# chao-ji/ldm_tf2

Hardware: AMD Instinct MI355X
Metric: images/sec (256x256, 200 DDIM steps, CFG=5) (higher is better)
Workload: dtype bf16

## Files before the change

ldm_tf2_amd/csrc/gemm.hip:

```cpp
#include "gemm_kernel.h"
#include "gemm3_kernel.h"
#include "gemm_tiles.h"

using namespace ldm_gemm_detail;

namespace {

__global__ __launch_bounds__(256) void splitk_epilogue_kernel(GemmArgs p) {
  const int nout = p.act == LDM_ACT_GEGLU ? p.N / 2 : p.N;
  const int64_t total = (int64_t)p.M * nout;
  for (int64_t idx = (int64_t)blockIdx.x * 256 + threadIdx.x; idx < total;
       idx += (int64_t)gridDim.x * 256) {
    const int m = (int)(idx / nout), c = (int)(idx - (int64_t)m * nout);
    if (p.act == LDM_ACT_GEGLU) {
      const int nv = (c >> 5) * 64 + (c & 31), ng = nv + 32;
      float a = 0.f, g = 0.f;
      for (int s = 0; s < p.split_k; ++s) {
        const float* ws = p.ws + ((int64_t)s * p.M + m) * p.N;
        a += ws[nv]; g += ws[ng];
      }
      epi_store(p, 0, m, c, epi_pre(p, m, nv, a) * gelu_erf_f(epi_pre(p, m, ng, g)));
    } else {
      float a = 0.f;
      for (int s = 0; s < p.split_k; ++s) a += p.ws[((int64_t)s * p.M + m) * p.N + c];
// ... 147 lines not shown
                        (p->split_k <= 0 && (!p->workspace || (size_t)split * p->M * p->N * 4 > p->workspace_bytes))))
        continue;
      const int kps = cdiv(ktiles, split);
      const double rounds = (double)(int64_t)((tiles * split + 256.0 * t.resident - 1) / (256.0 * t.resident));
      double us = rounds * (kps + t.overhead_steps) * t.step_us * f32x;
      if (!no_t2pref && t.prefer_over &&
          (double)m_tiles(p, kTiles[t.prefer_over].bm) * cdiv(p->N, kTiles[t.prefer_over].bn) * p->batch < 256.0)
        us *= kCoResidentPreference;
      if (split > 1) us += 3.0 + (double)p->M * p->N * 4.0 * (split + 1) / 3.0e6;
      if (us < best) { best = us; best_cfg = c; best_split = split; }
    }
  }
  if (p->split_k > 0 && p->batch == 1) best_split = p->split_k;
  const int twin = kTiles[best_cfg].halo_twin;
  if (tile_given) best_cfg = p->tile;
  else if (twin && halo_ring_ok(p) && p->N % kTiles[twin].bn == 0 && !p->out2 && !p->ln_out && !p->a2 &&
           ktiles / best_split >= kHaloTwinMinKtiles)
    best_cfg = twin;
  return {best_cfg, best_split, 0};
}

Plan final_plan(const ldm_gemm_params* p) {
  const int esize = elem_size(p);
  auto [cfg, split, kps] = choose(p, esize);
  if (p->ln_out) { cfg = kLnTile; split = 1; }
  if (p->ln_cs && !has(cfg, tPers)) {
    const bool wide_ok = p->act != LDM_ACT_GEGLU && p->N % kTiles[kLnFoldWideTile].bn == 0;
    cfg = wide_ok && (p->N % kTiles[kLnFoldTile].bn != 0 || p->tile == kLnFoldWideTile) ? kLnFoldWideTile : kLnFoldTile;
    split = 1;
  }
  if (p->out2 || has(cfg, tPers)) split = 1;
  const int ktiles = cdiv(p->K, 128 / esize);
  kps = cdiv(ktiles, split < 1 ? 1 : split);
  if (has(cfg, tHalo)) kps = cdiv(kps, 9) * 9;
  return {cfg, cdiv(ktiles, kps), kps};
}

int64_t a_extent(const ldm_gemm_params* p, int cols) {
  return (p->conv ? ((int64_t)p->B * p->H * p->W - 1) * p->lda + p->Cin : ((int64_t)p->M - 1) * p->lda + cols) * elem_size(p);
}
int64_t w_extent(const ldm_gemm_params* p) { return (int64_t)p->N * p->K * elem_size(p); }

template <typename Args>
Args common_args(const ldm_gemm_params* p) {
  Args a;
  memset(&a, 0, sizeof(a));
  a.a = (const char*)p->a; a.w = (const char*)p->w; a.bias = p->bias; a.addend = p->addend;
  a.residual = (const char*)p->residual; a.out = (char*)p->out;
  a.lda = p->lda; a.ldr = p->ldr; a.add_ld = p->add_ld; a.M = p->M; a.N = p->N; a.K = p->K;
  a.a_bytes = (uint32_t)a_extent(p, p->K - (p->a2 ? p->Cin2 : 0)); a.w_bytes = (uint32_t)w_extent(p);
  a.add_rows = p->add_rows > 0 ? p->add_rows : 1;
  a.conv = p->conv; a.H = p->H; a.W = p->W; a.Cin = p->Cin; a.OH = p->OH; a.OW = p->OW;
  a.stride = p->stride; a.upsample = p->upsample; a.pad = p->no_lead_pad ? 0 : 1; a.act = p->act;
  return a;
}

GemmArgs build_args(const ldm_gemm_params* p, Plan pl) {
  const int esize = elem_size(p), bke = 128 / esize;
  GemmArgs a = common_args<GemmArgs>(p);
  a.ws = (float*)p->workspace; a.ldc_m = p->ldc_m; a.ldc_n = p->ldc_n; a.batch = p->batch;
  a.stride_a = p->stride_a; a.stride_w = p->stride_w; a.stride_c = p->stride_c; a.stride_r = p->stride_r;
  a.out_dtype = p->out_dtype; a.alpha = p->alpha;
  a.ln_out = (char*)p->ln_out; a.ln_gamma = p->ln_gamma; a.ln_beta = p->ln_beta; a.ld_ln = p->ld_ln; a.ln_eps = p->ln_eps;
  a.out2 = (char*)p->out2; a.ld2 = p->ld2; a.stride2 = p->stride2; a.n_split = p->n_split; a.rows2 = p->rows2;
  a.ktiles = a.kt9 = cdiv(p->K, bke);
  if (p->a2) {
    a.a2 = (const char*)p->a2; a.lda2 = p->lda2; a.kt9 = (p->K - p->Cin2) / bke;
    a.a2_bytes = (uint32_t)((((int64_t)p->M - 1) * p->lda2 + p->Cin2) * esize);
  }
  a.vec_epilogue = vec_epilogue_ok(p);
  a.split_k = pl.split; a.ktiles_per_split = pl.kps;
  a.tiles_m = m_tiles(p, kTiles[pl.cfg].bm); a.tiles_n = cdiv(p->N, kTiles[pl.cfg].bn);
#ifdef LDM_TOOLS_BUILD
  { static const bool adj = getenv("LDM_UP2_PHASE_ADJACENT") != nullptr; a.phase_adjacent = adj; }
#endif
  return a;
}

int launch_reduce(const ldm_gemm_params* p, const GemmArgs& a, hipStream_t s) {
  const int nout = p->act == LDM_ACT_GEGLU ? p->N / 2 : p->N;
  const bool vec = a.vec_epilogue && ((uintptr_t)p->workspace % 16) == 0 && p->N % 4 == 0;
  int64_t total = vec ? (int64_t)p->M * (nout / 8) : (int64_t)p->M * nout;
  int blocks = (int)((total + 255) / 256);
  if (blocks > 4096) blocks = 4096;
  if (vec) hipLaunchKernelGGL(splitk_epilogue_vec_kernel, dim3(blocks), dim3(256), 0, s, a);
  else hipLaunchKernelGGL(splitk_epilogue_kernel, dim3(blocks), dim3(256), 0, s, a);
  return ldm_launch_status("ldm_gemm(splitk epilogue)");
}

int check_shape(const ldm_gemm_params* p) {
  LDM_CHECK_ARG(p && p->a && p->w && p->out, "ldm_gemm: null pointer");
  LDM_CHECK_ARG(p->dtype == LDM_F32 || p->dtype == LDM_BF16, "ldm_gemm: bad dtype %d", p->dtype);
  LDM_CHECK_ARG(p->out_dtype == LDM_F32 || p->out_dtype == LDM_BF16, "ldm_gemm: bad out_dtype");
  LDM_CHECK_ARG(p->M > 0 && p->N > 0 && p->K > 0 && p->batch > 0, "ldm_gemm: bad M/N/K/batch");
  const int esize = elem_size(p);
  const int epc = 16 / esize, bke = 8 * epc;
  LDM_CHECK_ARG(p->K % bke == 0, "ldm_gemm: K=%d must be a multiple of the K-tile (%d elements)", p->K, bke);
  LDM_CHECK_ARG(((uintptr_t)p->a % 16) == 0 && ((uintptr_t)p->w % 16) == 0,
                "ldm_gemm: a/w must be 16-byte aligned");
  LDM_CHECK_ARG(p->lda % epc == 0 && p->stride_a % epc == 0 && p->stride_w % epc == 0,
                "ldm_gemm: lda/stride_a/stride_w must be multiples of %d elements", epc);
  if (p->conv) {
    LDM_CHECK_ARG(p->Cin > 0 && p->Cin % bke == 0, "ldm_gemm(conv): Cin=%d must be a multiple of %d",
                  p->Cin, bke);
    if (p->upsample == 2) {
      LDM_CHECK_ARG(p->K == 4 * p->Cin, "ldm_gemm(conv): the phase form (upsample = 2) needs K == 4*Cin (K=%d Cin=%d)", p->K, p->Cin);
// ... 228 lines not shown
```

ldm_tf2_amd/csrc/gemm3_kernel.h:

```cpp
#pragma once
#include "gemm_kernel.h"

namespace ldm_gemm_detail {

struct Gemm3Args {
  const char* a;
  const char* w;
  const float* bias;
  const float* addend;
  const char* residual;
  char* out;
  int64_t lda, ldr, ldc, add_ld;
  uint32_t a_bytes, w_bytes;
  int M, N, K;
  int add_rows;
  int conv, H, W, Cin, OH, OW, stride, upsample, pad;
  int act;
  int ktiles;
  int panels;
  int ntiles;
  int nsplit;
  int tiles_per_wg;
  char* out_t;
  int64_t ld_t, stride_t;
  int rows_t;
  int n_split;
  int ntiles1;
  const float* ln_cs;
  float ln_eps;
#ifdef LDM_TOOLS_BUILD
  int dbg;
#endif
};

#ifdef LDM_TOOLS_BUILD
#define LDM_G3_DBG(p) ((p).dbg)
#else
#define LDM_G3_DBG(p) 0
#endif

constexpr int kEpiBias = 1, kEpiAdd = 2, kEpiRes = 4, kEpiTrans = 32, kEpiLn = 64, kEpiSplit = 128;
constexpr int epi_code(bool bias, bool add, bool res, int act) { return (bias ? 1 : 0) | (add ? 2 : 0) | (res ? 4 : 0) | (act << 3); }

#if defined(__HIP_DEVICE_COMPILE__)
template <int TN, int MODE, int EPI, bool TR>
__device__ __forceinline__ void gemm3_body(const Gemm3Args& p, char* smem, const int panel, const int nt_begin, const int ntl) {
  constexpr int BM = 256, BN = 32 * TN, WM = 4, WN = 2, NW = 8;
  constexpr int WTM = 64, WTN = 16 * TN, TM = 4;
  constexpr int NIB = BN / 8;
  constexpr int LA = BM / (8 * NW), LB = (NIB + NW - 1) / NW, LBF = NIB / NW;
  constexpr int NL = LA + LB;
  constexpr int ES = 2;
  constexpr int STAGE = (BM + BN) * 128;
  constexpr int NSTAGE = 3;
  constexpr int LNX = (EPI & 64) ? NW * 64 * 8 : 0;
  static_assert(NSTAGE * STAGE + LNX <= 160 * 1024, "LDS");
  typedef __attribute__((address_space(3))) void* lds_ptr;

  const int tid = threadIdx.x;
  const int lane = tid & 63;
  const int wave = __builtin_amdgcn_readfirstlane(tid >> 6);
  const int wm = wave / WN, wn = wave % WN;
  const int m0 = panel * BM;
  const int nk = p.ktiles;
  const int S = ntl * nk;

  const __amdgpu_buffer_rsrc_t rsA =
      __builtin_amdgcn_make_buffer_rsrc(const_cast<char*>(p.a), 0, p.a_bytes, 0x00020000);
  const __amdgpu_buffer_rsrc_t rsW =
      __builtin_amdgcn_make_buffer_rsrc(const_cast<char*>(p.w), 0, p.w_bytes, 0x00020000);

  int a_base[LA], a_mask[LA], a_aux[LA];
#pragma unroll
  for (int i = 0; i < LA; ++i) {
    const int row = (i * NW + wave) * 8 + (lane >> 3);
    const int ck = (lane & 7) ^ ((row >> 1) & 7);
    const int m = m0 + row;
    a_base[i] = MODE == 0 ? (int)kOOB : 0; a_mask[i] = 0; a_aux[i] = 0;
    if (m < p.M) {
      if constexpr (MODE != 0) {
        const int ohw = p.OH * p.OW;
        const int b = m / ohw, rem = m - b * ohw;
        const int oy = rem / p.OW, ox = rem - oy * p.OW;
        const int iy0 = oy * p.stride - p.pad, ix0 = ox * p.stride - p.pad;
// ... 134 lines not shown
                                                                __builtin_bit_cast(bf16x8, fb[kg][j]), acc[i][j], 0, 0, 0);
          else
            acc[i][j] = __builtin_amdgcn_mfma_f32_16x16x32_bf16(__builtin_bit_cast(bf16x8, fb[kg][j]),
                                                                __builtin_bit_cast(bf16x8, fa[kg][i]), acc[i][j], 0, 0, 0);
        }
    __builtin_amdgcn_s_setprio(0);
  };

  [[maybe_unused]] float ln_s = 0.f, ln_q = 0.f;
  [[maybe_unused]] auto ln_accum = [&](const char* cS) {
    if constexpr ((EPI & kEpiLn) != 0) {
      typedef __bf16 bf2 __attribute__((ext_vector_type(2)));
      const int row = wm * WTM + lane;
      const char* base = cS + row * 128;
      const int rot = row >> 1;
      const bf2 one = __builtin_bit_cast(bf2, 0x3f803f80u);
#pragma unroll
      for (int j = 0; j < 8; j += 2) {
        const u32x4 c0 = *(const u32x4*)(base + (((j + rot) & 7) << 4));
        const u32x4 c1 = *(const u32x4*)(base + (((j + 1 + rot) & 7) << 4));
#pragma unroll
        for (int e = 0; e < 4; ++e) {
          const uint32_t w0 = c0[e], w1 = c1[e];
          const bf2 a0 = __builtin_bit_cast(bf2, w0), a1 = __builtin_bit_cast(bf2, w1);
          ln_s = __builtin_amdgcn_fdot2_f32_bf16(a0, one, ln_s, false);
          ln_q = __builtin_amdgcn_fdot2_f32_bf16(a0, a0, ln_q, false);
          ln_s = __builtin_amdgcn_fdot2_f32_bf16(a1, one, ln_s, false);
          ln_q = __builtin_amdgcn_fdot2_f32_bf16(a1, a1, ln_q, false);
        }
      }
    }
  };

  [[maybe_unused]] auto ln_publish = [&]() {
    if constexpr ((EPI & kEpiLn) != 0) {
      ldm_f32x2 v = {ln_s, ln_q};
      *(ldm_f32x2*)(smem + NSTAGE * STAGE + (wave * 64 + lane) * 8) = v;
      asm volatile("s_waitcnt lgkmcnt(0)" ::: "memory");
    }
  };
  [[maybe_unused]] auto ln_combine = [&]() {
    if constexpr ((EPI & kEpiLn) != 0) {
      const ldm_f32x2 o = *(const ldm_f32x2*)(smem + NSTAGE * STAGE + ((wave ^ 1) * 64 + lane) * 8);
      ln_s += o[0]; ln_q += o[1];
    }
  };

  constexpr bool HB = (EPI & kEpiBias) != 0, HA = (EPI & kEpiAdd) != 0, HR = (EPI & kEpiRes) != 0;
  constexpr int ACT = (EPI >> 3) & 3;
  constexpr bool LN = (EPI & kEpiLn) != 0;
  static_assert(!LN || (MODE == 0 && HB), "LayerNorm fold: plain rows, with the folded bias");
  constexpr bool GEGLU = ACT == LDM_ACT_GEGLU;
  static_assert(!GEGLU || TN == 4, "GEGLU: the wave tile must be one 64-row block of the interleaved weights");
  auto epilogue = [&](int tl) {
    if (LDM_G3_DBG(p) & 2) return;
    const int n_w = (nt_begin + tl) * BN + wn * WTN;
    const int g = lh;
    [[maybe_unused]] float ln_mu = 0.f, ln_r = 0.f;
    if constexpr (LN) {
      const float ik = 1.0f / (float)p.K;
      ln_mu = ln_s * ik;
      const float ex2 = ln_q * ik;
      ln_r = rsqrtf(fmaxf(__builtin_fmaf(-ln_mu, ln_mu, ex2), 0.f) + p.ln_eps);
    }
    if constexpr (TR) {
      const int n_t = SPLIT ? n_w - p.n_split : n_w;
      const int col2 = lane >> 2, pc = lane & 3;
      const int src = (16 * ((pc >> 1) | ((pc & 1) << 1)) + col2) * 4;
#pragma unroll
      for (int ip = 0; ip < TM; ip += 2) {
        const int mrow = m0 + wm * WTM + 16 * ip + 8 * pc;
        const bool valid = mrow < p.M && !(LDM_G3_DBG(p) & 1);
        const int mc = valid ? mrow : 0;
        const int smp = mc / p.rows_t, tok = mc - smp * p.rows_t;
        bf16_t* obase = (bf16_t*)p.out_t + (int64_t)smp * p.stride_t + tok;
        [[maybe_unused]] float rmu[2][4], rrs[2][4];
        if constexpr (LN) {
#pragma unroll
          for (int h = 0; h < 2; ++h)
#pragma unroll
            for (int r = 0; r < 4; ++r) {
              rmu[h][r] = __shfl(ln_mu, 16 * (ip + h) + 4 * g + r, 64);
              rrs[h][r] = __shfl(ln_r, 16 * (ip + h) + 4 * g + r, 64);
            }
        }
#pragma unroll
        for (int j = 0; j < TN; ++j) {
          if constexpr (LN) {
            const float cs = p.ln_cs[n_w + 16 * j + lr], bb = p.bias[n_w + 16 * j + lr];
#pragma unroll
            for (int h = 0; h < 2; ++h)
#pragma unroll
              for (int r = 0; r < 4; ++r)
                acc[ip + h][j][r] = __builtin_fmaf(rrs[h][r], acc[ip + h][j][r], __builtin_fmaf(-rrs[h][r] * rmu[h][r], cs, bb));
          }
          const uint32_t x0 = pack_bf2(acc[ip][j][0], acc[ip][j][1]), x1 = pack_bf2(acc[ip][j][2], acc[ip][j][3]);
          const uint32_t y0 = pack_bf2(acc[ip + 1][j][0], acc[ip + 1][j][1]), y1 = pack_bf2(acc[ip + 1][j][2], acc[ip + 1][j][3]);
          const auto s0 = __builtin_amdgcn_permlane16_swap(x0, y0, false, false);
          const auto s1 = __builtin_amdgcn_permlane16_swap(x1, y1, false, false);
          u32x4 o;
          o[0] = (uint32_t)__builtin_amdgcn_ds_bpermute(src, (int)s0[0]);
          o[1] = (uint32_t)__builtin_amdgcn_ds_bpermute(src, (int)s1[0]);
          o[2] = (uint32_t)__builtin_amdgcn_ds_bpermute(src, (int)s0[1]);
          o[3] = (uint32_t)__builtin_amdgcn_ds_bpermute(src, (int)s1[1]);
          if (valid) *(u32x4*)(obase + (int64_t)(n_t + 16 * j + col2) * p.ld_t) = o;
        }
      }
      return;
    }
    f32x4 bv[TN];
    if constexpr (HB) {
#pragma unroll
      for (int j = 0; j < TN; ++j) bv[j] = *(const f32x4*)(p.bias + n_w + 16 * j + 4 * g);
    }
    [[maybe_unused]] f32x4 csv[TN];
    if constexpr (LN) {
#pragma unroll
      for (int j = 0; j < TN; ++j) csv[j] = *(const f32x4*)(p.ln_cs + n_w + 16 * j + 4 * g);
    }
    constexpr int NOB = GEGLU ? TN / 2 : TN;
    const int n_o = GEGLU ? (n_w >> 1) : n_w;
    [[maybe_unused]] u32x2 rva[TM][NOB];
    if constexpr (HR) {
#pragma unroll
      for (int i = 0; i < TM; ++i) {
        const int m = m0 + wm * WTM + 16 * i + lr;
        const bf16_t* rr = (const bf16_t*)p.residual + (int64_t)(m < p.M ? m : p.M - 1) * p.ldr + n_o + 4 * g;
#pragma unroll
        for (int j = 0; j < NOB; ++j) rva[i][j] = *(const u32x2*)(rr + 16 * j);
      }
    }
#pragma unroll
    for (int i = 0; i < TM; ++i) {
      const int m = m0 + wm * WTM + 16 * i + lr;
      const bool valid = m < p.M;
      const int mc = valid ? m : p.M - 1;
      f32x4 av[TN];
      if constexpr (HA) {
        const float* ad = p.addend + (int64_t)(mc / p.add_rows) * p.add_ld + n_w + 4 * g;
#pragma unroll
        for (int j = 0; j < TN; ++j) av[j] = *(const f32x4*)(ad + 16 * j);
      }
      u32x2 rv[NOB];
      if constexpr (HR) {
#pragma unroll
        for (int j = 0; j < NOB; ++j) rv[j] = rva[i][j];
      }
      [[maybe_unused]] float mu_i = 0.f, rs_i = 0.f;
      [[maybe_unused]] float nm_i = 0.f;
      if constexpr (LN) {
        mu_i = __shfl(ln_mu, 16 * i + lr, 64);
        rs_i = __shfl(ln_r, 16 * i + lr, 64);
        nm_i = -rs_i * mu_i;
      }
      auto block = [&](int j, float (&v)[4]) {
#pragma unroll
        for (int r = 0; r < 4; ++r) v[r] = acc[i][j][r];
        if constexpr (LN) {
#pragma unroll
          for (int r = 0; r < 4; ++r) v[r] = __builtin_fmaf(rs_i, v[r], __builtin_fmaf(nm_i, csv[j][r], bv[j][r]));
        } else if constexpr (HB) {
#pragma unroll
          for (int r = 0; r < 4; ++r) v[r] += bv[j][r];
        }
        if constexpr (HA) {
#pragma unroll
          for (int r = 0; r < 4; ++r) v[r] += av[j][r];
        }
      };
      auto finish = [&](int jo, float (&v)[4], uint32_t (&pk)[2]) {
        if constexpr (HR) {
          v[0] += __uint_as_float(rv[jo][0] << 16); v[1] += __uint_as_float(rv[jo][0] & 0xffff0000u);
          v[2] += __uint_as_float(rv[jo][1] << 16); v[3] += __uint_as_float(rv[jo][1] & 0xffff0000u);
        }
        pk[0] = pack_bf2(v[0], v[1]);
        pk[1] = pack_bf2(v[2], v[3]);
      };
      uint32_t pk[NOB][2];
      if constexpr (GEGLU) {
#pragma unroll
        for (int j = 0; j < 2; ++j) {
          float v[4], gt[4];
          block(j, v);
// ... 6 lines not shown
#pragma unroll
        for (int j = 0; j < TN; ++j) {
          float v[4];
          block(j, v);
          if constexpr (ACT == LDM_ACT_GELU) {
#pragma unroll
            for (int r = 0; r < 4; ++r) v[r] = gelu_erf_f(v[r]);
          } else if constexpr (ACT == LDM_ACT_SILU) {
#pragma unroll
            for (int r = 0; r < 4; ++r) v[r] = silu_f(v[r]);
          }
          finish(j, v, pk[j]);
        }
      }
      const int row2 = lane >> 2, pc = lane & 3;
      const int src = (16 * ((pc >> 1) | ((pc & 1) << 1)) + row2) * 4;
      const int m2 = m0 + wm * WTM + 16 * i + row2;
      const bool valid2 = m2 < p.M && !(LDM_G3_DBG(p) & 1);
      bf16_t* orow2 = (bf16_t*)p.out + (int64_t)(valid2 ? m2 : 0) * p.ldc + n_o;
#pragma unroll
      for (int j = 0; j + 1 < NOB; j += 2) {
        const auto s0 = __builtin_amdgcn_permlane16_swap(pk[j][0], pk[j + 1][0], false, false);
        const auto s1 = __builtin_amdgcn_permlane16_swap(pk[j][1], pk[j + 1][1], false, false);
        u32x4 o;
        o[0] = (uint32_t)__builtin_amdgcn_ds_bpermute(src, (int)s0[0]);
        o[1] = (uint32_t)__builtin_amdgcn_ds_bpermute(src, (int)s1[0]);
        o[2] = (uint32_t)__builtin_amdgcn_ds_bpermute(src, (int)s0[1]);
        o[3] = (uint32_t)__builtin_amdgcn_ds_bpermute(src, (int)s1[1]);
        if (valid2) *(u32x4*)(orow2 + 16 * j + 8 * pc) = o;
      }
      if constexpr (NOB & 1) {
        const int src1 = (16 * pc + row2) * 4;
        u32x2 o;
        o[0] = (uint32_t)__builtin_amdgcn_ds_bpermute(src1, (int)pk[NOB - 1][0]);
        o[1] = (uint32_t)__builtin_amdgcn_ds_bpermute(src1, (int)pk[NOB - 1][1]);
        if (valid2) *(u32x2*)(orow2 + 16 * (NOB - 1) + 4 * pc) = o;
      }
    }
  };

  int is_tl = 0, is_kt = 0;
  auto issue_next = [&](int stage) {
    if (!(LDM_G3_DBG(p) & 8)) issue_tile(is_tl, is_kt, stage);
    if (++is_kt == nk) { is_kt = 0; ++is_tl; }
  };
  issue_next(0);
  if (S > 1) issue_next(1);
  int st = 0, ck = 0, ctl = 0;
  const bool late = wave >= NW / 2;
  auto wait_step = [&](int s) {
    if (s + 1 < S && (LDM_G3_DBG(p) & 16)) {
      if (b_last) asm volatile("s_waitcnt vmcnt(%0)" ::"n"(LB) : "memory");
      else asm volatile("s_waitcnt vmcnt(%0)" ::"n"(LB - 1) : "memory");
    } else if (s + 1 < S) {
      if (b_last) asm volatile("s_waitcnt vmcnt(%0)" ::"n"(NL) : "memory");
      else asm volatile("s_waitcnt vmcnt(%0)" ::"n"(NL - 1) : "memory");
    } else {
      asm volatile("s_waitcnt vmcnt(0)" ::: "memory");
    }
  };
  if (!late) {
    for (int s = 0; s < S; ++s) {
      wait_step(s);
      __builtin_amdgcn_s_barrier();
      if constexpr (LN) { if (s == nk) ln_combine(); }
      if (ck == 0 && s > 0) { epilogue(ctl - 1); zero_acc(); }
      int sn = st + 2; sn = sn >= NSTAGE ? sn - NSTAGE : sn;
      if (s + 2 < S) issue_next(sn);
      read_frags(smem + st * STAGE);
      if constexpr (LN) {
        if (ctl == 0) {
          if ((ck & 1) == wn) ln_accum(smem + st * STAGE);
          if (ck == nk - 1) ln_publish();
        }
      }
      multiply(0);
      st = st + 1 == NSTAGE ? 0 : st + 1;
      if (++ck == nk) { ck = 0; ++ctl; }
    }
  } else {
    for (int s = 0; s < S; ++s) {
      wait_step(s);
      __builtin_amdgcn_s_barrier();
      if (s > 0) multiply(1);
      if constexpr (LN) { if (s == nk) ln_combine(); }
      if (ck == 0 && s > 0) { epilogue(ctl - 1); zero_acc(); }
      int sn = st + 2; sn = sn >= NSTAGE ? sn - NSTAGE : sn;
      if (s + 2 < S) issue_next(sn);
      read_frags(smem + st * STAGE);
      if constexpr (LN) {
        if (ctl == 0) {
          if ((ck & 1) == wn) ln_accum(smem + st * STAGE);
          if (ck == nk - 1) ln_publish();
        }
      }
      st = st + 1 == NSTAGE ? 0 : st + 1;
      if (++ck == nk) { ck = 0; ++ctl; }
      asm volatile("s_waitcnt lgkmcnt(0)" ::: "memory");
      __builtin_amdgcn_sched_barrier(0);
    }
    multiply(1);
  }
  if constexpr (LN) {
    if (ntl == 1) {
      __builtin_amdgcn_s_barrier();
      ln_combine();
    }
  }
  epilogue(ntl - 1);
}
#endif

template <int TN, int MODE, int EPI>
__global__ __launch_bounds__(512) void gemm3_kernel(Gemm3Args p) {
#if defined(__HIP_DEVICE_COMPILE__)
  constexpr int BM = 256, BN = 32 * TN;
  constexpr int LNX = (EPI & 64) ? 8 * 64 * 8 : 0;
  __shared__ __attribute__((aligned(16))) char smem[3 * (BM + BN) * 128 + LNX];
  int bid = blockIdx.x;
  {
    const int nwg = gridDim.x;
    const int q = nwg >> 3, r = nwg & 7, x = bid & 7;
    bid = (x < r ? x * (q + 1) : r * (q + 1) + (x - r) * q) + (bid >> 3);
  }
  const int panel = bid / p.nsplit, sp = bid - panel * p.nsplit;
  if constexpr ((EPI & kEpiSplit) != 0) {
    const int nt_begin = sp * p.tiles_per_wg;
    const int nt_end = min(p.ntiles, nt_begin + p.tiles_per_wg);
    const int a_end = min(nt_end, p.ntiles1);
    if (nt_begin < a_end) gemm3_body<TN, MODE, EPI, false>(p, smem, panel, nt_begin, a_end - nt_begin);
    const int b_begin = max(nt_begin, p.ntiles1);
    if (b_begin < nt_end) {
      if (nt_begin < a_end) __syncthreads();
      gemm3_body<TN, MODE, EPI, true>(p, smem, panel, b_begin, nt_end - b_begin);
    }
  } else {
    const int nt_begin = sp * p.tiles_per_wg;
    const int ntl = min(p.ntiles, nt_begin + p.tiles_per_wg) - nt_begin;
    if (ntl > 0)
      gemm3_body<TN, MODE, EPI, (EPI & kEpiTrans) != 0>(p, smem, panel, nt_begin, ntl);
  }
#endif
}

template <int MODE>
bool launch_gemm3(int tn, int epi, const Gemm3Args& a, dim3 grid, hipStream_t s);
bool launch_gemm3_ln(int tn, int epi, const Gemm3Args& a, dim3 grid, hipStream_t s);

}
```

ldm_tf2_amd/csrc/gemm_kernel.h:

```cpp
#pragma once
#include "common.h"
#include <stdlib.h>

namespace ldm_gemm_detail {


struct GemmArgs {
  const char* a;
  const char* w;
  const float* bias;
  const float* addend;
  const char* residual;
  char* out;
  float* ws;
  int64_t lda, ldr, ldc_m, ldc_n;
  int64_t stride_a, stride_w, stride_c, stride_r;
  int64_t add_ld;
  uint32_t a_bytes, w_bytes;
  int M, N, K, batch;
  int add_rows;
  int conv, H, W, Cin, OH, OW, stride, upsample, pad;
  int act, out_dtype;
  int split_k, ktiles_per_split, ktiles;
  int tiles_m, tiles_n;
  int vec_epilogue;
  float alpha;
  char* ln_out;
  const float* ln_gamma;
  const float* ln_beta;
  int64_t ld_ln;
  float ln_eps;
  char* out2;
  int64_t ld2, stride2;
  int n_split, rows2;
  const char* a2;
  int64_t lda2;
  uint32_t a2_bytes;
  int kt9;
  int phase_adjacent;
};

constexpr uint32_t kOOB = 0x80000000u;

__device__ __forceinline__ void mma32(f32x16& acc, const u32x4& a, const u32x4& b, bf16_t) {
  acc = __builtin_amdgcn_mfma_f32_32x32x16_bf16(__builtin_bit_cast(bf16x8, a),
                                                __builtin_bit_cast(bf16x8, b), acc, 0, 0, 0);
}
__device__ __forceinline__ void mma32(f32x16& acc, const u32x4& a, const u32x4& b, float) {
#pragma unroll
  for (int j = 0; j < 4; ++j)
    acc = __builtin_amdgcn_mfma_f32_32x32x2f32(__uint_as_float(a[j]), __uint_as_float(b[j]), acc,
                                               0, 0, 0);
}

__device__ __forceinline__ uint32_t pick6(int j, uint32_t a0, uint32_t a1, uint32_t a2, uint32_t a3, uint32_t a4, uint32_t a5) {
  uint32_t v = a0;
  v = j == 1 ? a1 : v;
  v = j == 2 ? a2 : v;
  v = j == 3 ? a3 : v;
  v = j == 4 ? a4 : v;
  v = j == 5 ? a5 : v;
  return v;
}

__device__ __forceinline__ float epi_pre(const GemmArgs& p, int m, int n, float acc) {
  float v = acc * p.alpha;
  if (p.bias) v += p.bias[n];
  if (p.addend) v += p.addend[(int64_t)(m / p.add_rows) * p.add_ld + n];
  return v;
}

__device__ __forceinline__ void epi_store(const GemmArgs& p, int bz, int m, int ncol, float v) {
  const int64_t off = (int64_t)bz * p.stride_c + (int64_t)m * p.ldc_m + (int64_t)ncol * p.ldc_n;
  if (p.out_dtype == LDM_BF16) {
    if (p.residual)
      v += bf2f(((const bf16_t*)p.residual)[(int64_t)bz * p.stride_r + (int64_t)m * p.ldr + ncol]);
    ((bf16_t*)p.out)[off] = f2bf(v);
  } else {
    if (p.residual)
      v += ((const float*)p.residual)[(int64_t)bz * p.stride_r + (int64_t)m * p.ldr + ncol];
    ((float*)p.out)[off] = v;
  }
}

__device__ __forceinline__ float apply_act(int act, float v) {
  if (act == LDM_ACT_GELU) return gelu_erf_f(v);
  if (act == LDM_ACT_SILU) return silu_f(v);
  return v;
}

template <typename T, int BM, int BN, int WM, int WN, int MODE, int MF = 0, int ST = 0, int NS = 0>
__global__ __launch_bounds__(WM* WN * 64) void gemm_kernel(GemmArgs p) {
#if defined(__HIP_DEVICE_COMPILE__)
// ... 441 lines not shown
#pragma unroll
          for (int e = 0; e < 4; ++e)
            v[e] = apply_act(p.act, epi_pre(p, min(m + e, p.M - 1), n, acc[i][j][r4 * 4 + e]));
          const int64_t off = (int64_t)(m / p.rows2) * p.stride2 + (int64_t)(n - p.n_split) * p.ld2 + (m % p.rows2);
          if (p.out_dtype == LDM_BF16) {
            u32x2 pk; pk[0] = pack_bf2(v[0], v[1]); pk[1] = pack_bf2(v[2], v[3]);
            *(u32x2*)((bf16_t*)p.out2 + off) = pk;
          } else {
            f32x4 pk = {v[0], v[1], v[2], v[3]};
            *(f32x4*)((float*)p.out2 + off) = pk;
          }
        }
      }
    return;
  }
  if (p.split_k > 1) {
    float* ws = p.ws + (int64_t)split * p.M * p.N;
#pragma unroll
    for (int i = 0; i < TM; ++i)
#pragma unroll
      for (int j = 0; j < TN; ++j) {
        const int n = nb + j * MB;
        if (n >= p.N) continue;
#pragma unroll
        for (int r = 0; r < NR; ++r) {
          const int m = mb + i * MB + rowoff(r);
          if (m < Mrows) ws[(int64_t)orow(m) * p.N + n] = acc[i][j][r];
        }
      }
    return;
  }

  if (p.vec_epilogue) {
    float* sC = (float*)smem;
    const bool geglu = p.act == LDM_ACT_GEGLU;
    constexpr int PCOLS = BN / 8;
    const int pcols = geglu ? PCOLS / 2 : PCOLS;
    const int npieces = EROWS * pcols;
    const int nout = geglu ? p.N / 2 : (p.out2 ? p.n_split : p.N);
#pragma unroll
   for (int ep = 0; ep < ESPLIT; ++ep) {
    if (ep > 0) __syncthreads();
    if ((wm * WTM) / EROWS == ep) {
#pragma unroll
      for (int i = 0; i < TM; ++i)
#pragma unroll
        for (int j = 0; j < TN; ++j)
#pragma unroll
          for (int r = 0; r < NR; ++r) {
            const int row = wm * WTM - ep * EROWS + i * MB + rowoff(r) + 4 * lh;
            sC[row * BN + wn * WTN + j * MB + lr] = acc[i][j][r] * p.alpha;
          }
    }
    __syncthreads();
    for (int c = tid; c < npieces; c += NT) {
      const int row = c / pcols, pc = c - row * pcols;
      int m = m0 + ep * EROWS + row;
      int ncol, lcol;
      if (geglu) {
        const int oc = pc * 8;
        lcol = (oc >> 5) * 64 + (oc & 31);
        ncol = (n0 >> 1) + oc;
      } else {
        lcol = pc * 8;
        ncol = n0 + lcol;
      }
      if (m >= Mrows || ncol >= nout) continue;
      m = orow(m);
      float v[8];
      {
        const f32x4 x0 = *(const f32x4*)(sC + row * BN + lcol);
        const f32x4 x1 = *(const f32x4*)(sC + row * BN + lcol + 4);
#pragma unroll
        for (int e = 0; e < 4; ++e) { v[e] = x0[e]; v[4 + e] = x1[e]; }
      }
      const int nlog = geglu ? n0 + lcol : ncol;
      if (p.bias) {
        const f32x4 b0 = *(const f32x4*)(p.bias + nlog), b1 = *(const f32x4*)(p.bias + nlog + 4);
#pragma unroll
        for (int e = 0; e < 4; ++e) { v[e] += b0[e]; v[4 + e] += b1[e]; }
      }
      if (p.addend) {
        const float* ad = p.addend + (int64_t)(m / p.add_rows) * p.add_ld + nlog;
        const f32x4 a0 = *(const f32x4*)ad, a1 = *(const f32x4*)(ad + 4);
#pragma unroll
        for (int e = 0; e < 4; ++e) { v[e] += a0[e]; v[4 + e] += a1[e]; }
      }
      if (geglu) {
        float g[8];
        const f32x4 x0 = *(const f32x4*)(sC + row * BN + lcol + 32);
        const f32x4 x1 = *(const f32x4*)(sC + row * BN + lcol + 36);
#pragma unroll
        for (int e = 0; e < 4; ++e) { g[e] = x0[e]; g[4 + e] = x1[e]; }
        if (p.bias) {
          const f32x4 b0 = *(const f32x4*)(p.bias + nlog + 32), b1 = *(const f32x4*)(p.bias + nlog + 36);
#pragma unroll
          for (int e = 0; e < 4; ++e) { g[e] += b0[e]; g[4 + e] += b1[e]; }
        }
#pragma unroll
        for (int e = 0; e < 8; ++e) v[e] *= gelu_erf_f(g[e]);
      } else if (p.act != LDM_ACT_NONE) {
#pragma unroll
        for (int e = 0; e < 8; ++e) v[e] = apply_act(p.act, v[e]);
      }
      const int64_t ooff = (int64_t)bz * p.stride_c + (int64_t)m * p.ldc_m + ncol;
      const int64_t roff = (int64_t)bz * p.stride_r + (int64_t)m * p.ldr + ncol;
      if (p.out_dtype == LDM_BF16) {
        if (p.residual) {
          float rr[8];
          chunk_to_f32(*(const u32x4*)((const bf16_t*)p.residual + roff), rr, bf16_t());
#pragma unroll
          for (int e = 0; e < 8; ++e) v[e] += rr[e];
        }
        *(u32x4*)((bf16_t*)p.out + ooff) = f32_to_chunk(v, bf16_t());
      } else {
        if (p.residual) {
          const f32x4 r0 = *(const f32x4*)((const float*)p.residual + roff);
          const f32x4 r1 = *(const f32x4*)((const float*)p.residual + roff + 4);
#pragma unroll
          for (int e = 0; e < 4; ++e) { v[e] += r0[e]; v[4 + e] += r1[e]; }
        }
        f32x4 o0 = {v[0], v[1], v[2], v[3]}, o1 = {v[4], v[5], v[6], v[7]};
        *(f32x4*)((float*)p.out + ooff) = o0;
        *(f32x4*)((float*)p.out + ooff + 4) = o1;
      }
      if (p.ln_out) {
        if (p.out_dtype == LDM_BF16) {
#pragma unroll
          for (int e = 0; e < 8; ++e) v[e] = bf2f(f2bf(v[e]));
        }
        f32x4 o0 = {v[0], v[1], v[2], v[3]}, o1 = {v[4], v[5], v[6], v[7]};
        *(f32x4*)(sC + row * BN + lcol) = o0;
        *(f32x4*)(sC + row * BN + lcol + 4) = o1;
      }
    }
    if (p.ln_out) {
      __syncthreads();
      const bool act = lane < BN / 8;
      float gm[8], bt[8];
#pragma unroll
      for (int e = 0; e < 8; ++e) { gm[e] = act ? p.ln_gamma[lane * 8 + e] : 0.f; bt[e] = act ? p.ln_beta[lane * 8 + e] : 0.f; }
      for (int row = wave; row < EROWS; row += NW) {
        const int m = m0 + ep * EROWS + row;
        if (m >= p.M) break;
        float f[8];
#pragma unroll
        for (int e = 0; e < 8; ++e) f[e] = 0.f;
        if (act) {
          const f32x4 x0 = *(const f32x4*)(sC + row * BN + lane * 8), x1 = *(const f32x4*)(sC + row * BN + lane * 8 + 4);
#pragma unroll
          for (int e = 0; e < 4; ++e) { f[e] = x0[e]; f[4 + e] = x1[e]; }
        }
        float s = 0.f;
#pragma unroll
        for (int e = 0; e < 8; ++e) s += f[e];
        const float mean = wave_sum(s) * (1.0f / BN);
        float q = 0.f;
#pragma unroll
        for (int e = 0; e < 8; ++e) { const float d = f[e] - mean; q += act ? d * d : 0.f; }
        const float rstd = rsqrtf(wave_sum(q) * (1.0f / BN) + p.ln_eps);
        if (act) {
          float y[8];
#pragma unroll
          for (int e = 0; e < 8; ++e) y[e] = (f[e] - mean) * rstd * gm[e] + bt[e];
          const int64_t loff = (int64_t)m * p.ld_ln + lane * 8;
          if (p.out_dtype == LDM_BF16) {
            *(u32x4*)((bf16_t*)p.ln_out + loff) = f32_to_chunk(y, bf16_t());
          } else {
            f32x4 o0 = {y[0], y[1], y[2], y[3]}, o1 = {y[4], y[5], y[6], y[7]};
            *(f32x4*)((float*)p.ln_out + loff) = o0;
            *(f32x4*)((float*)p.ln_out + loff + 4) = o1;
// ... 84 lines not shown
```

ldm_tf2_amd/ops.py:

```python
from __future__ import annotations

import ctypes as C
import os
import threading

import torch

from . import _lib
from ._lib import ACT_GEGLU, ACT_GELU, ACT_NONE, ACT_SILU, BF16, F32, GemmParams, check, lib

__all__ = [
    "ACT_NONE", "ACT_GELU", "ACT_GEGLU", "ACT_SILU", "F32", "BF16", "code", "linear", "conv3x3",
    "bmm_nt", "conv3x3_small", "groupnorm", "layernorm", "softmax_rows", "attention",
    "time_embedding", "gemv", "cfg_ddim_update", "cfg_ddim_update_masked", "cfg_plms_update", "q_sample",
    "philox_u32", "normal_fill", "q_sample_rng", "cfg_ddim_update_rng", "cfg_plms_update_rng", "cfg_ms_update",
    "cfg_ms_update_rng", "cfg_sched_update", "cfg_ddim_invert_update", "window_gather", "window_fold", "window_gather_ex", "window_fold_ex", "wrap_pad", "resize_nhwc", "resample_nhwc", "latent_preview", "xattn_map", "xattn_map_supported",
    "eps_contrast_accum", "contrast_mask", "contrast_mask_supported", "store_row", "pushpull_fill", "pushpull_workspace", "mask_feather", "mask_feather_workspace", "keep_stats", "paste_back", "post_quant", "vq_nearest", "embedding",
    "minmax_u8", "cast",
]

_TORCH_DT = {torch.float32: F32, torch.bfloat16: BF16}
_byref = C.byref
_WS = {}
_WS_BYTES = 96 << 20
# ... 264 lines not shown
  return st


def finish(pending):
  if pending is None or pending.done:
    return
  check(lib.ldm_gemm_reduce(C.byref(pending.p), _stream()), "ldm_gemm_reduce")
  pending.done = True
  _outstanding().pop(pending.ws.data_ptr(), None)


def _launch(p: GemmParams, device, defer=None):
  ws = workspace(device)
  if ws.data_ptr() in _outstanding():
    raise RuntimeError("ldm_gemm: this workspace still holds the slabs of a deferred split-K product "
                       "(ops.finish it, or let the GroupNorm that follows consume it, first)")
  p.workspace, p.workspace_bytes = ws.data_ptr(), ws.numel()
  planned = resolve_plan(p)
  while True:
    split = defer is not None and lib.ldm_gemm_splits(C.byref(p)) > 1
    p.defer_reduce = int(split)
    st = lib.ldm_gemm(C.byref(p), _stream())
    if st in (_lib.ERR_ARG, _lib.ERR_WORKSPACE) and planned:
      planned, p.tile, p.split_k = False, 0, 0
      continue
    check(st, "ldm_gemm")
    if split:
      _outstanding()[ws.data_ptr()] = pend = PendingReduce(p, defer[0], ws, defer[1])
      return pend
    return None


def _gemm_deferred(p: GemmParams, device, out, keep):
  return _launch(p, device, (out, keep))


def _gemm(p: GemmParams, device):
  _launch(p, device)


def linear_ln_supported(n_out, dtype):
  return bool(lib.ldm_gemm_ln_supported(int(n_out), code(dtype)))


def _row_params(x, wt, out, M, N, K, bias=None, addend=None, add_rows=0, residual=None, x2=None, act=ACT_NONE,
                alpha=1.0, tile=0, split_k=0):
  p = GemmParams()
  p.a, p.w, p.out = _ptr(x), _ptr(wt), _ptr(out)
  p.bias = _ptr(_f32(bias, "bias"))
  p.addend = _ptr(_f32(addend, "addend"))
  p.residual = _ptr(residual)
  if residual is not None:
    assert residual.dtype == out.dtype
    p.ldr = row_ld(residual)
  p.lda, p.ldc_m, p.ldc_n = row_ld(x), row_ld(out), 1
  p.M, p.N, p.K, p.batch = M, N, K, 1
  if x2 is not None:
    assert x2.dtype == x.dtype and x2.numel() // x2.shape[-1] == M
    p.a2, p.lda2, p.Cin2 = _ptr(x2), row_ld(x2), x2.shape[-1]
  if addend is not None:
    p.add_rows = add_rows
    p.add_ld = addend.stride(0) if (addend.dim() == 2 and addend.shape[0] > 1) else 0
  p.act, p.dtype, p.out_dtype, p.alpha = act, code(x.dtype), code(out.dtype), alpha
  p.tile, p.split_k = tile, split_k
  return p


def linear(x, wt, out, bias=None, act=ACT_NONE, residual=None, addend=None, add_rows=0,
           alpha=1.0, tile=0, split_k=0, ln=None, out2=None, ln_fold=None, x2=None, defer_reduce=False):
  K1, K2 = x.shape[-1], (0 if x2 is None else x2.shape[-1])
  K, N, M = K1 + K2, wt.shape[0], x.numel() // K1
  assert wt.shape[1] == K and wt.is_contiguous() and wt.dtype == x.dtype
  p = _row_params(x, wt, out, M, N, K, bias, addend, add_rows if add_rows > 0 else M, residual, x2, act, alpha, tile, split_k)
  if out2 is not None:
    assert out2.dtype == out.dtype and out2.dim() == 3 and out2.stride(2) == 1 and M % out2.shape[0] == 0
    assert out.shape[-1] + out2.shape[1] == N and out2.shape[2] >= M // out2.shape[0]
    p.out2, p.n_split, p.rows2 = _ptr(out2), out.shape[-1], M // out2.shape[0]
    p.ld2, p.stride2 = out2.stride(1), out2.stride(0)
  if ln is not None:
    gamma, beta, ln_out, eps = ln
    assert ln_out.dtype == out.dtype and tuple(ln_out.shape) == tuple(out.shape)
    p.ln_out, p.ld_ln, p.ln_eps = _ptr(ln_out), row_ld(ln_out), float(eps)
    p.ln_gamma, p.ln_beta = _ptr(_f32(gamma, "ln gamma")), _ptr(_f32(beta, "ln beta"))
  if ln_fold is not None:
    cs, eps = ln_fold
    assert bias is not None and tuple(cs.shape) == (N,) and cs.is_contiguous()
    p.ln_cs, p.ln_eps = _ptr(_f32(cs, "ln_fold column sums")), float(eps)
  if defer_reduce:
    return _gemm_deferred(p, x.device, out, (x, wt, bias, addend, residual, x2))
  _gemm(p, x.device)
  return out


def linear_t_shape_supported(dtype, K, N, rows, ld, stride):
  return (dtype == torch.bfloat16 and K % 64 == 0 and (N % 128 == 0 or N % 160 == 0) and rows % 32 == 0 and
          ld % 8 == 0 and stride % 8 == 0)


def linear_t_supported(x, wt, out_t):
  K, N = x.shape[-1], wt.shape[0]
  M = x.numel() // K
  G = out_t.shape[0]
  return (out_t.dtype == x.dtype and M % G == 0 and out_t.stride(2) == 1 and
          linear_t_shape_supported(x.dtype, K, N, M // G, out_t.stride(1), out_t.stride(0)))


# ... 807 lines not shown
```

Baseline: 9.306.

## Prefetch residual tiles early to overlap epilogue loads with main loop

In the gemm3 kernel, residual values for the next tile are loaded during the second-to-last K iteration and held in registers, with the vmcnt waits adjusted so these loads stay outstanding while the final MMA steps run. In the generic GEMM epilogue, residual chunks are prefetched into registers before the shared-memory barrier instead of being read inside the store loop. The aim is to hide residual-read latency in epilogues. In exchange it uses more registers, makes the waitcnt accounting more fragile, and now requires residual and output to be different buffers, which is enforced by a new assert in the Python wrapper.

```diff
diff --git a/ldm_tf2_amd/csrc/gemm.hip b/ldm_tf2_amd/csrc/gemm.hip
--- a/ldm_tf2_amd/csrc/gemm.hip
+++ b/ldm_tf2_amd/csrc/gemm.hip
@@ -223,6 +223,9 @@
   a.add_rows = p->add_rows > 0 ? p->add_rows : 1;
   a.conv = p->conv; a.H = p->H; a.W = p->W; a.Cin = p->Cin; a.OH = p->OH; a.OW = p->OW;
   a.stride = p->stride; a.upsample = p->upsample; a.pad = p->no_lead_pad ? 0 : 1; a.act = p->act;
+#ifdef LDM_TOOLS_BUILD
+  a.res_late = getenv("LDM_EPI_RESIDUAL_LATE") != nullptr;
+#endif
   return a;
 }
 
diff --git a/ldm_tf2_amd/csrc/gemm3_kernel.h b/ldm_tf2_amd/csrc/gemm3_kernel.h
--- a/ldm_tf2_amd/csrc/gemm3_kernel.h
+++ b/ldm_tf2_amd/csrc/gemm3_kernel.h
@@ -30,6 +30,7 @@
   float ln_eps;
 #ifdef LDM_TOOLS_BUILD
   int dbg;
+  int res_late;
 #endif
 };
 
@@ -270,6 +271,30 @@
   static_assert(!LN || (MODE == 0 && HB), "LayerNorm fold: plain rows, with the folded bias");
   constexpr bool GEGLU = ACT == LDM_ACT_GEGLU;
   static_assert(!GEGLU || TN == 4, "GEGLU: the wave tile must be one 64-row block of the interleaved weights");
+  constexpr bool HRES = (EPI & kEpiRes) != 0 && !TR;
+  constexpr int NOBR = ((EPI >> 3) & 3) == LDM_ACT_GEGLU ? TN / 2 : TN;
+  constexpr int NRES = HRES ? TM * NOBR : 0;
+  [[maybe_unused]] u32x2 rva[TM][NOBR];
+  [[maybe_unused]] const bool res_early = HRES && nk >= 3 && !LDM_RES_LATE(p) && !LDM_G3_DBG(p);
+  if constexpr (HRES) {
+#pragma unroll
+    for (int i = 0; i < TM; ++i)
+#pragma unroll
+      for (int j = 0; j < NOBR; ++j) rva[i][j] = u32x2{0u, 0u};
+  }
+  [[maybe_unused]] auto residual_load = [&](int tl) {
+    if constexpr (HRES) {
+      const int n_o = ((nt_begin + tl) * BN + wn * WTN) >> (NOBR != TN ? 1 : 0);
+#pragma unroll
+      for (int i = 0; i < TM; ++i) {
+        const int m = m0 + wm * WTM + 16 * i + lr;
+        const bf16_t* rr = (const bf16_t*)p.residual + (int64_t)(m < p.M ? m : p.M - 1) * p.ldr + n_o + 4 * lh;
+#pragma unroll
+        for (int j = 0; j < NOBR; ++j) rva[i][j] = *(const u32x2*)(rr + 16 * j);
+      }
+    }
+  };
+
   auto epilogue = [&](int tl) {
     if (LDM_G3_DBG(p) & 2) return;
     const int n_w = (nt_begin + tl) * BN + wn * WTN;
@@ -338,15 +363,9 @@
     }
     constexpr int NOB = GEGLU ? TN / 2 : TN;
     const int n_o = GEGLU ? (n_w >> 1) : n_w;
-    [[maybe_unused]] u32x2 rva[TM][NOB];
+    static_assert(NOB == NOBR, "residual blocks");
     if constexpr (HR) {
-#pragma unroll
-      for (int i = 0; i < TM; ++i) {
-        const int m = m0 + wm * WTM + 16 * i + lr;
-        const bf16_t* rr = (const bf16_t*)p.residual + (int64_t)(m < p.M ? m : p.M - 1) * p.ldr + n_o + 4 * g;
-#pragma unroll
-        for (int j = 0; j < NOB; ++j) rva[i][j] = *(const u32x2*)(rr + 16 * j);
-      }
+      if (!res_early) residual_load(tl);
     }
 #pragma unroll
     for (int i = 0; i < TM; ++i) {
@@ -459,6 +478,13 @@
     if (s + 1 < S && (LDM_G3_DBG(p) & 16)) {
       if (b_last) asm volatile("s_waitcnt vmcnt(%0)" ::"n"(LB) : "memory");
       else asm volatile("s_waitcnt vmcnt(%0)" ::"n"(LB - 1) : "memory");
+    } else if (res_early && ck == nk - 1) {
+      if (s + 1 < S) {
+        if (b_last) asm volatile("s_waitcnt vmcnt(%0)" ::"n"(NL + NRES) : "memory");
+        else asm volatile("s_waitcnt vmcnt(%0)" ::"n"(NL - 1 + NRES) : "memory");
+      } else {
+        asm volatile("s_waitcnt vmcnt(%0)" ::"n"(NRES) : "memory");
+      }
     } else if (s + 1 < S) {
       if (b_last) asm volatile("s_waitcnt vmcnt(%0)" ::"n"(NL) : "memory");
       else asm volatile("s_waitcnt vmcnt(%0)" ::"n"(NL - 1) : "memory");
@@ -466,6 +492,7 @@
       asm volatile("s_waitcnt vmcnt(0)" ::: "memory");
     }
   };
+  static_assert(NL + NRES < 64, "vmcnt is a 6-bit count");
   if (!late) {
     for (int s = 0; s < S; ++s) {
       wait_step(s);
@@ -474,6 +501,7 @@
       if (ck == 0 && s > 0) { epilogue(ctl - 1); zero_acc(); }
       int sn = st + 2; sn = sn >= NSTAGE ? sn - NSTAGE : sn;
       if (s + 2 < S) issue_next(sn);
+      if (res_early && s > 0 && ck == nk - 2) residual_load(ctl);
       read_frags(smem + st * STAGE);
       if constexpr (LN) {
         if (ctl == 0) {
@@ -485,6 +513,7 @@
       st = st + 1 == NSTAGE ? 0 : st + 1;
       if (++ck == nk) { ck = 0; ++ctl; }
     }
+    if constexpr (HRES) epilogue(ntl - 1);
   } else {
     for (int s = 0; s < S; ++s) {
       wait_step(s);
@@ -494,6 +523,7 @@
       if (ck == 0 && s > 0) { epilogue(ctl - 1); zero_acc(); }
       int sn = st + 2; sn = sn >= NSTAGE ? sn - NSTAGE : sn;
       if (s + 2 < S) issue_next(sn);
+      if (res_early && s > 0 && ck == nk - 2) residual_load(ctl);
       read_frags(smem + st * STAGE);
       if constexpr (LN) {
         if (ctl == 0) {
@@ -507,6 +537,7 @@
       __builtin_amdgcn_sched_barrier(0);
     }
     multiply(1);
+    if constexpr (HRES) epilogue(ntl - 1);
   }
   if constexpr (LN) {
     if (ntl == 1) {
@@ -514,7 +545,7 @@
       ln_combine();
     }
   }
-  epilogue(ntl - 1);
+  if constexpr (!HRES) epilogue(ntl - 1);
 }
 #endif
 
diff --git a/ldm_tf2_amd/csrc/gemm_kernel.h b/ldm_tf2_amd/csrc/gemm_kernel.h
--- a/ldm_tf2_amd/csrc/gemm_kernel.h
+++ b/ldm_tf2_amd/csrc/gemm_kernel.h
@@ -38,7 +38,16 @@
   uint32_t a2_bytes;
   int kt9;
   int phase_adjacent;
+#ifdef LDM_TOOLS_BUILD
+  int res_late;
+#endif
 };
+
+#ifdef LDM_TOOLS_BUILD
+#define LDM_RES_LATE(p) ((p).res_late != 0)
+#else
+#define LDM_RES_LATE(p) false
+#endif
 
 constexpr uint32_t kOOB = 0x80000000u;
 
@@ -586,11 +595,10 @@
             sC[row * BN + wn * WTN + j * MB + lr] = acc[i][j][r] * p.alpha;
           }
     }
-    __syncthreads();
-    for (int c = tid; c < npieces; c += NT) {
-      const int row = c / pcols, pc = c - row * pcols;
-      int m = m0 + ep * EROWS + row;
-      int ncol, lcol;
+    auto piece = [&](int c, int& row, int& m, int& ncol, int& lcol) {
+      row = c / pcols;
+      const int pc = c - row * pcols;
+      m = m0 + ep * EROWS + row;
       if (geglu) {
         const int oc = pc * 8;
         lcol = (oc >> 5) * 64 + (oc & 31);
@@ -599,6 +607,31 @@
         lcol = pc * 8;
         ncol = n0 + lcol;
       }
+    };
+    constexpr int PPT = (EROWS * PCOLS + NT - 1) / NT;
+    constexpr int RPF = PPT < 8 ? PPT : 8;
+    u32x4 rpre[RPF];
+    const bool res_pre = p.residual != nullptr && !LDM_RES_LATE(p);
+    const int rpieces = p.out_dtype == LDM_BF16 ? RPF : RPF / 2;
+    if (res_pre) {
+      const int rstep = p.out_dtype == LDM_BF16 ? 1 : 2;
+#pragma unroll
+      for (int q = 0; q < RPF; ++q) {
+        int row, m, ncol, lcol;
+        piece(min(tid + (q / rstep) * NT, npieces - 1), row, m, ncol, lcol);
+        const int64_t roff = (int64_t)bz * p.stride_r + (int64_t)orow(min(m, Mrows - 1)) * p.ldr + min(ncol, nout - 8);
+        if (p.out_dtype == LDM_BF16) rpre[q] = *(const u32x4*)((const bf16_t*)p.residual + roff);
+        else rpre[q] = *(const u32x4*)((const float*)p.residual + roff + 4 * (q & 1));
+      }
+    }
+    __syncthreads();
+#pragma unroll
+    for (int k = 0; k < PPT; ++k) {
+      __builtin_amdgcn_sched_barrier(0);
+      const int c = tid + k * NT;
+      if (c >= npieces) break;
+      int row, m, ncol, lcol;
+      piece(c, row, m, ncol, lcol);
       if (m >= Mrows || ncol >= nout) continue;
       m = orow(m);
       float v[8];
@@ -639,18 +672,19 @@
       }
       const int64_t ooff = (int64_t)bz * p.stride_c + (int64_t)m * p.ldc_m + ncol;
       const int64_t roff = (int64_t)bz * p.stride_r + (int64_t)m * p.ldr + ncol;
+      const bool pre = res_pre && k < rpieces;
       if (p.out_dtype == LDM_BF16) {
         if (p.residual) {
           float rr[8];
-          chunk_to_f32(*(const u32x4*)((const bf16_t*)p.residual + roff), rr, bf16_t());
+          chunk_to_f32(pre ? rpre[k < RPF ? k : 0] : *(const u32x4*)((const bf16_t*)p.residual + roff), rr, bf16_t());
 #pragma unroll
           for (int e = 0; e < 8; ++e) v[e] += rr[e];
         }
         *(u32x4*)((bf16_t*)p.out + ooff) = f32_to_chunk(v, bf16_t());
       } else {
         if (p.residual) {
-          const f32x4 r0 = *(const f32x4*)((const float*)p.residual + roff);
-          const f32x4 r1 = *(const f32x4*)((const float*)p.residual + roff + 4);
+          const f32x4 r0 = pre ? __builtin_bit_cast(f32x4, rpre[2 * k + 1 < RPF ? 2 * k : 0]) : *(const f32x4*)((const float*)p.residual + roff);
+          const f32x4 r1 = pre ? __builtin_bit_cast(f32x4, rpre[2 * k + 1 < RPF ? 2 * k + 1 : 0]) : *(const f32x4*)((const float*)p.residual + roff + 4);
 #pragma unroll
           for (int e = 0; e < 4; ++e) { v[e] += r0[e]; v[4 + e] += r1[e]; }
         }
diff --git a/ldm_tf2_amd/ops.py b/ldm_tf2_amd/ops.py
--- a/ldm_tf2_amd/ops.py
+++ b/ldm_tf2_amd/ops.py
@@ -340,6 +340,7 @@
   p.residual = _ptr(residual)
   if residual is not None:
     assert residual.dtype == out.dtype
+    assert residual.data_ptr() != out.data_ptr(), "ldm_gemm: residual and out must be different tensors"
     p.ldr = row_ld(residual)
   p.lda, p.ldc_m, p.ldc_n = row_ld(x), row_ld(out), 1
   p.M, p.N, p.K, p.batch = M, N, K, 1
```

Measured after the change: 9.247. No clear change (-0.6%).
